# Hevagog/as-cops-and-thieves

Hardware: AMD Instinct MI355X
Metric: env-steps/sec (whole node) at 4096 parallel envs, 2v1 agents, 64-ray sensors (higher is better)
Workload: dtype f64; 1 GPU; 2 cops vs 1 thieves, labyrinth map (30 hull walls / 119 planes), 4096 envs per GPU, 64 rays/agent, dt=1/60, max_step_count=400, Philox random actions, auto-reset; envs_per_gpu=4096, rays=64, agents=3, map=labyrinth, parallelism=env-sharded x1, no data-path collective, episodes_reset_per_gpu=32768, burn_in_steps=600

## Files before the change

### as_cops_and_thieves_amd/csrc/cat_sim_scheduler.h

```cpp
template <class D>
__device__ __forceinline__ Lds carve(const Params &p, char *smem, const MapDesc &md, int slot, int wave)
{
    Lds L;
    const int S = md.S, P = md.P, W = p.wpb;
    L.bb = reinterpret_cast<const double *>(smem);
    L.planes = L.bb + kBB * S;
    L.p32 = reinterpret_cast<const float *>(L.planes + 8 * P);
    L.fc = reinterpret_cast<const int *>(L.planes + geo_rest_doubles(md));
    L.fp = L.fc + S;
    L.rayd = reinterpret_cast<const double *>(smem + p.lds_map_bytes - 16 * D::R(p));
    L.ctrl = reinterpret_cast<int *>(smem + p.lds_map_bytes);
    char *w = smem + p.lds_map_bytes + ctrl_bytes(W) + slot * p.lds_env_bytes;
    const int A = D::A(p), R = D::R(p), NPs = D::NP(p) > 0 ? D::NP(p) : 1;
    L.rec = w;
    double *d = reinterpret_cast<double *>(w);
    L.pos = d; d += 2 * A; L.vel = d; d += 2 * A; L.vb = d; d += 2 * A; L.tc = d; d += 2 * A;
    L.leaf = d; d += 4 * A;
    L.cnt = reinterpret_cast<int *>(d);
    d = reinterpret_cast<double *>(w + D::hot_bytes(p));
    L.wjn = d; d += A * kK; L.pjn = d; d += NPs;
    {
        int *ri = reinterpret_cast<int *>(d);
        L.wsh = ri; ri += A * kK; L.wag = ri; ri += A * kK; L.pag = ri;
    }
// ... 297 lines not shown
            else {
                PHASE(pc, 9);
                physics_env<D>(Ls, p, uni(K->md.S), lane, pc);
                PHASE(pc, 10);
            }
            __builtin_amdgcn_fence(__ATOMIC_RELEASE, "workgroup");
            int d = 0;
            if (lane == 0) {
                d = __hip_atomic_fetch_add(&ctrl[4 * slot + 1], 1, __ATOMIC_RELAXED, __HIP_MEMORY_SCOPE_WORKGROUP);
                c = __hip_atomic_fetch_add(&ctrl[4 * slot + 0], 1, __ATOMIC_RELAXED, __HIP_MEMORY_SCOPE_WORKGROUP);
            }
            d = uni(d); c = uni(c);
            if (d == last_unit) fin_mask |= 1u << slot;
        }
    }
    PHASE(pc, 16);
    if (fin_mask) __builtin_amdgcn_fence(__ATOMIC_ACQUIRE, "workgroup");
    PHASE(pc, 21);
#ifdef CAT_PHASE_TIMING
    bool wb_first = true;
#endif
    while (fin_mask) {
        const int lane = opaque_v(lane0);
        const Params &p = *(const Params *)launder((ParamsK)pp0);
        const LaunchArgs &la = *(const LaunchArgs *)launder(lap0);
        int *const ctrl = reinterpret_cast<int *>(smem + p.lds_map_bytes);
        const BlockDesc *const K = block_desc_lds(smem, p, W);
        const int slot = uni(__builtin_ctz(fin_mask));
        fin_mask &= fin_mask - 1;
        const Lds Ls = carve<D>(p, smem, K->md, slot, wave);
        const int e_s = uni(ctrl[4 * slot + 3]);
        const int step2 = uni(Ls.flags[0]), captured2 = uni(Ls.flags[1]), timeout2 = uni(Ls.flags[2]), rcount = uni(Ls.flags[3]);
        PHASE(pc, 22);
#ifdef CAT_PHASE_TIMING
        asm volatile("s_waitcnt vmcnt(0)" ::: "memory");
        if (wb_first) PHASE(pc, 23); else PHASE(pc, 3);
        wb_first = false;
#endif
        slot_writeback<D>(Ls, p, la, e_s, (long long)e_s, lane, tick, true, step2, captured2, timeout2, rcount, cop_lut, thief_lut, pc);
    }
}

template <class D>
__device__ __forceinline__ void spawn_and_reset(const Lds &L, const Params &p, const LaunchArgs &la, const MapDesc &md,
                                                int env, unsigned rc, int lane);

template <class D>
__device__ __forceinline__ int slot_front(const Lds &L, ParamsK pk, const LaunchArgs &la, const MapDesc &md, const GridDesc &gd,
                                          int env, int lane, int act_pref, unsigned long long synth_tick, int n_fan, PhaseClock &pc)
{
    int captured, timeout, step;
    SetupRow row;
    {
        const Params &p = *(const Params *)launder(pk);
        const int S = md.S, A = D::A(p);
        row = setup_row(L.pos, p, gd, lane, A);
        step = uni(L.cnt[0]) + 1;
        captured = termination_captured<D>(L, p, S, lane);
        timeout = (!captured && step >= p.max_step) ? 1 : 0;
        copy_snapshot(L, A, lane);

        if (lane < A) {
            const int i = lane;
            const double m_inv = 1.0 / p.mass;
            int act;
            if (la.actions) act = act_pref;
            else { unsigned rnd[4]; philox_env(p, env, (unsigned)synth_tick, (unsigned)i, 0xAC710u, rnd); act = (int)(rnd[0] & 3u); }
            if ((unsigned)act > 3u) atomicOr(p.err_word, CAT_DEVERR_BAD_ACTION);
            double jx = 0.0, jy = 0.0;
            if (act == 0) jx = -p.impulse; else if (act == 1) jy = p.impulse;
            else if (act == 2) jx = p.impulse; else if (act == 3) jy = -p.impulse;
            double vx = L.vel[2 * i] + jx * m_inv, vy = L.vel[2 * i + 1] + jy * m_inv;
            double len = sqrt(vx * vx + vy * vy);
            if (len > p.max_speed) { vx = vx / len * p.max_speed; vy = vy / len * p.max_speed; }
            L.vel[2 * i] = vx; L.vel[2 * i + 1] = vy;
        }
        wave_sync();
        PHASE(pc, 2);
    }
    int n_units, rcount = -1, step_store = step;
    {
        const Params &p = *(const Params *)launder(pk);
        n_units = n_fan + 1;
        if (la.auto_reset && (captured || timeout)) {
            physics_env<D>(L, p, uni(md.S), lane, pc);
            rcount = uni(L.cnt[1]) + 1;
            spawn_and_reset<D>(L, p, la, md, env, (unsigned)rcount, lane);
            wave_sync();
            copy_snapshot(L, D::A(p), lane);
            n_units -= 1; step_store = 0;
            row = setup_row(L.fpos, p, gd, lane, D::A(p));
        }
    }
    {
        const Params &p = *(const Params *)launder(pk);
        agent_setup<D>(L, p, gd, lane, row);
        PHASE(pc, 4);
    }
    if (lane == 0) { L.flags[0] = step_store; L.flags[1] = captured; L.flags[2] = timeout; L.flags[3] = rcount; }
    return n_units;
}

constexpr unsigned kRwFinished = 0xFFFFFFFFu;
__device__ __forceinline__ unsigned rw_make(int epoch, int n_units) { return ((unsigned)epoch << 14) | ((unsigned)n_units << 7); }
__device__ __forceinline__ int rw_next(unsigned w) { return (int)(w & 127u); }
__device__ __forceinline__ int rw_units(unsigned w) { return (int)((w >> 7) & 127u); }
__device__ __forceinline__ int rw_epoch(unsigned w) { return (int)(w >> 14); }

__device__ __forceinline__ void lds_release() { __builtin_amdgcn_fence(__ATOMIC_RELEASE, "workgroup", "local"); }
__device__ __forceinline__ void lds_acquire() { __builtin_amdgcn_fence(__ATOMIC_ACQUIRE, "workgroup", "local"); }

template <class D, bool kOneTick>
__device__ __forceinline__ void rollout_body(const Params *__restrict__ pp0, const LaunchArgs &la0)
{
    extern __shared__ __align__(16) char smem[];
    const int lane0 = threadIdx.x % kLanes;
    const int wave = uni(threadIdx.x / kLanes);
    const LaunchArgsK lap0 = kernarg_launch_args();
    PhaseClock pc;
    WSPREAD(0); WSPREAD(4);
    int env, T, W;
    GAS const float *lut_c, *lut_t;
    {
        int uniform;
        const Params q = prologue_params(kernarg_prologue(), uniform);
        const Params &p = *(const Params *)(ParamsK)pp0;
        lut_c = G(q.cop_lut); lut_t = G(q.thief_lut);
        const int lane = lane0;
        W = uni((int)(blockDim.x / kLanes));
        T = kOneTick ? 1 : la0.T;
        WSPREAD(6);
        int *const ctrl = reinterpret_cast<int *>(smem + q.lds_map_bytes);
        BlockDesc bd0;
        prologue_env_desc(q, uniform, W, wave, env, bd0);
        const MapDesc &md0 = bd0.md;
#ifdef CAT_WAVE_SPREAD
        { int e_ = env, s_ = md0.S; asm volatile("" : "+s"(e_), "+v"(s_)); WSPREAD(7); }
#endif
        if (lane < 4) ctrl[4 * wave + lane] = lane == 3 ? env : ((lane == 0 && env < 0) ? (int)kRwFinished : 0);
        StateRegs sregs;
        fetch_state<D>(sregs, q, env, lane);
        stage_map<D>(q, smem, md0, &bd0, const_cast<BlockDesc *>(block_desc_lds(smem, q, W)));
        PHASE(pc, 0);
        WSPREAD(1);
        if (env >= 0) {
            const Lds L = carve<D>(q, smem, md0, wave, wave);
            commit_state<D>(L, sregs, q, lane);
            load_cold<D>(L, p, env, lane);
            PHASE(pc, 1);
        }
    }
    int pend = env >= 0 ? wave : -1, pend_t = 0;
    int hint = wave;
    for (;;) {
        if (pend >= 0) {
            const int lane = opaque_v(lane0);
            const Params &p = *(const Params *)launder((ParamsK)pp0);
            const LaunchArgs &la = *(const LaunchArgs *)launder(lap0);
            int *const ctrl = reinterpret_cast<int *>(smem + p.lds_map_bytes);
            const BlockDesc *const K = block_desc_lds(smem, p, W);
            const int slot = pend, t = pend_t;
            pend = -1;
            SSPREAD(slot, 0);
            const int e_s = uni(ctrl[4 * slot + 3]);
            const Lds Ls = carve<D>(p, smem, K->md, slot, wave);
            int ap = 0;
            if (la.actions && lane < D::A(p)) ap = la.actions[((size_t)t * p.N + e_s) * D::A(p) + lane];
            if (lane == 0) ctrl[4 * slot + 1] = 0;
            const int n_fan = fan_units<D>(p, unit_span<D, kOneTick>(p, K->gd));
#ifndef CAT_ABL_NOFRONT
            const int n2 = slot_front<D>(Ls, (ParamsK)pp0, la, K->md, K->gd, e_s, lane, ap, la.synth_tick + (unsigned long long)t, n_fan, pc);
#else
            const int n2 = n_fan + 1;
            if (lane == 0) { Ls.flags[0] = 1; Ls.flags[1] = 0; Ls.flags[2] = 0; Ls.flags[3] = -1; }
            (void)ap;
#endif
            lds_release();
            if (lane == 0) __hip_atomic_store((unsigned *)&ctrl[4 * slot], rw_make(t + 1, n2), __ATOMIC_RELAXED, __HIP_MEMORY_SCOPE_WORKGROUP);
            hint = slot;
            PHASE(pc, 3);
            WSPREAD(2); SSPREAD(slot, 1);
        }
        int slot, unit, n_units, t;
        {
            const int lane = opaque_v(lane0);
            int *const ctrl = reinterpret_cast<int *>(smem + launder((ParamsK)pp0)->lds_map_bytes);
            unsigned w_l = kRwFinished;
            if (lane < W) w_l = __hip_atomic_load((unsigned *)&ctrl[4 * lane], __ATOMIC_RELAXED, __HIP_MEMORY_SCOPE_WORKGROUP);
            const unsigned open = (unsigned)__ballot(rw_next(w_l) < rw_units(w_l));
            if (open == 0u) {
                if (__ballot(kOneTick ? (w_l == 0u) : (w_l != kRwFinished)) == 0ull) break;
                __builtin_amdgcn_s_sleep(4);
                PHASE(pc, 21);
                continue;
            }
            unsigned key = 0xFFFFFFFFu;
            if (rw_next(w_l) < rw_units(w_l)) key = ((unsigned)rw_epoch(w_l) << 5) | (unsigned)((lane - hint) & 31);
#define CAT_ROW_MIN(SH) { const unsigned o_ = (unsigned)__builtin_amdgcn_update_dpp((int)key, (int)key, 0x120 + SH, 0xF, 0xF, false); key = o_ < key ? o_ : key; }
            CAT_ROW_MIN(8) CAT_ROW_MIN(4) CAT_ROW_MIN(2) CAT_ROW_MIN(1)
#undef CAT_ROW_MIN
            slot = uni((hint + (int)(key & 31u)) & 31);
            const unsigned wv = (unsigned)__builtin_amdgcn_readlane((int)w_l, slot);
            unsigned seen = wv;
            if (lane == 0)
                __hip_atomic_compare_exchange_strong((unsigned *)&ctrl[4 * slot], &seen, wv + 1u, __ATOMIC_RELAXED, __ATOMIC_RELAXED,
                                                     __HIP_MEMORY_SCOPE_WORKGROUP);
            if ((unsigned)uni((int)seen) != wv) continue;
            lds_acquire();
            hint = slot;
            unit = rw_next(wv); n_units = rw_units(wv); t = rw_epoch(wv) - 1;
            PHASE(pc, 22);
        }
        bool fin;
        {
            const int lane = opaque_v(lane0);
            const Params &p = *(const Params *)launder((ParamsK)pp0);
            const LaunchArgs &la = *(const LaunchArgs *)launder(lap0);
            int *const ctrl = reinterpret_cast<int *>(smem + p.lds_map_bytes);
            const BlockDesc *const K = block_desc_lds(smem, p, W);
            const int e_s = uni(ctrl[4 * slot + 3]);
            const Lds Ls = carve<D>(p, smem, K->md, slot, wave);
            const long long eo = (long long)t * p.N + e_s;
            const int gsz = unit_span<D, kOneTick>(p, K->gd);
            SSPREAD(slot, 2 + 2 * unit);
            if (unit < fan_units<D>(p, gsz)) {
#ifndef CAT_ABL_NOFAN
                if constexpr (D::kFan == 1) fan_group<D>(Ls, p, la, K->gd, eo, lane, uni(K->md.S), K->md.cmax, 1, unit, gsz, pc);
                else {
                    const int nch = D::A(p) * ((D::R(p) + kLanes - 1) / kLanes), c0 = unit * gsz, nq = nch - c0 < gsz ? nch - c0 : gsz;
                    unsigned chunks = D::kFixed ? (1u << nq) - 1u : 1u;
                    if (D::kFixed && gsz > 1) chunks = fan_slot<D>(Ls, p, la, K->gd, eo, lane, uni(K->md.S), K->md.cmax, 1, c0, nq, pc);
                    while (chunks) {
                        const int q = uni(__builtin_ctz(chunks));
                        chunks &= chunks - 1;
                        fan_chunk<D>(Ls, p, la, K->gd, eo, lane, uni(K->md.S), K->md.cmax, 1, c0 + q, pc);
                    }
                }
#endif
            } else {
                PHASE(pc, 9);
#ifndef CAT_ABL_NOPHYS
                physics_env<D>(Ls, p, uni(K->md.S), lane, pc);
#endif
                PHASE(pc, 10);
            }
            lds_release();
            SSPREAD(slot, 3 + 2 * unit);
            int d = 0;
            if (lane == 0) d = __hip_atomic_fetch_add(&ctrl[4 * slot + 1], 1, __ATOMIC_RELAXED, __HIP_MEMORY_SCOPE_WORKGROUP);
            fin = uni(d) == n_units - 1;
            PHASE(pc, 23);
        }
        if (!fin) continue;
        {
            const int lane = opaque_v(lane0);
            const Params &p = *(const Params *)launder((ParamsK)pp0);
            const LaunchArgs &la = *(const LaunchArgs *)launder(lap0);
            int *const ctrl = reinterpret_cast<int *>(smem + p.lds_map_bytes);
            const BlockDesc *const K = block_desc_lds(smem, p, W);
            lds_acquire();
            PHASE(pc, 16);
            SSPREAD(slot, 12);
            const int e_s = uni(ctrl[4 * slot + 3]);
            const Lds Ls = carve<D>(p, smem, K->md, slot, wave);
            const long long eo = (long long)t * p.N + e_s;
            const int step2 = uni(Ls.flags[0]), captured2 = uni(Ls.flags[1]), timeout2 = uni(Ls.flags[2]), rcount = uni(Ls.flags[3]);
            const bool last = t + 1 >= T;
#ifndef CAT_ABL_NOWB
            slot_writeback<D>(Ls, p, la, e_s, eo, lane, 1, last, step2, captured2, timeout2, rcount, lut_c, lut_t, pc);
#else
            (void)eo; (void)step2; (void)captured2; (void)timeout2; (void)rcount; (void)la;
#endif
            wave_sync();
            SSPREAD(slot, 13);
            if (!last) { pend = slot; pend_t = t + 1; }
            else if (lane == 0) __hip_atomic_store((unsigned *)&ctrl[4 * slot], kRwFinished, __ATOMIC_RELAXED, __HIP_MEMORY_SCOPE_WORKGROUP);
        }
    }
    PHASE(pc, 11);
    WSPREAD(3); WSPREAD(5);
    pc.flush(lane0);
}

template <class D>
__global__ __launch_bounds__(kMaxWaves *kLanes) void rollout_kernel(const Params *__restrict__ pp0, const LaunchArgs la0, const Prologue)
{
    rollout_body<D, false>(pp0, la0);
}

template <class D>
__global__ __launch_bounds__(kMaxWaves *kLanes) void step_kernel(const Params *__restrict__ pp0, const LaunchArgs la0, const Prologue)
{
    rollout_body<D, true>(pp0, la0);
}

#ifdef CAT_WB_COUNTS
__device__ unsigned long long g_wb_counts[8];
extern "C" int cat_debug_wb_counts(unsigned long long *out8, int reset)
{
    unsigned long long h[8];
    if (hipMemcpyFromSymbol(h, HIP_SYMBOL(g_wb_counts), sizeof h) != hipSuccess) return -1;
    for (int i = 0; i < 8; i++) out8[i] = h[i];
    if (reset) { memset(h, 0, sizeof h); if (hipMemcpyToSymbol(HIP_SYMBOL(g_wb_counts), h, sizeof h) != hipSuccess) return -1; }
    return 0;
}
#endif
template <class T> __device__ __forceinline__ T *slot_ptr(T *p0, int sl, int envb) { return (T *)((char *)const_cast<typename std::remove_const<T>::type *>(p0) + sl * envb); }
constexpr unsigned kPoolValid = 0x80000000u;
constexpr double kPoolEmptyRows = 0.05;
#ifndef CAT_POOL_ROUND
#define CAT_POOL_ROUND 60
#endif
#ifndef CAT_POOL_MIN_PARTIAL
#define CAT_POOL_MIN_PARTIAL 40
#endif
#ifndef CAT_POOL_PATIENCE
#define CAT_POOL_PATIENCE 3
#endif
constexpr int kPoolRound = CAT_POOL_ROUND;
constexpr int kPoolMinPartial = CAT_POOL_MIN_PARTIAL;
constexpr int kPoolPatience = CAT_POOL_PATIENCE;
#ifdef CAT_FAULT_INJECT
constexpr int kSpinLimit = 1 << 14;
#else
constexpr int kSpinLimit = 1 << 22;
#endif
__device__ __forceinline__ int *pool_ctl(char *smem, const Params &p, int W) { return reinterpret_cast<int *>(smem + p.lds_map_bytes + 16 * W + kWgConstBytes - 8); }
static_assert(sizeof(BlockDesc) <= kWgConstBytes - 8, "the pool counters live behind the BlockDesc");

template <bool kExact>
__device__ __forceinline__ int ring_pos(const Params &p, unsigned i)
{
    if constexpr (!kExact) return (int)(i & (unsigned)p.pool_mask);
    const unsigned t = __umulhi(p.pool_magic, i);
    const unsigned q = (t + ((i - t) >> 1)) >> p.pool_shift;
    return (int)(i - q * (unsigned)(p.pool_mask + 1));
}

template <class D, bool kExact>
__device__ __forceinline__ int pool_sort(const Lds &L, const Params &p, const LaunchArgs &la, const GridDesc &gd, long long env, int slot, int lane,
                                         int *pctl, unsigned long long *pool)
{
    const int A = D::A(p), R = D::R(p);
    const unsigned d_empty = f64_to_f16(p.ray_length);
    const unsigned long long lt_mask = (1ull << lane) - 1ull;
    const int cpa = (R + kLanes - 1) / kLanes, nch = A * cpa;
    const int my_cell = lane < A ? L.acell[lane] : -1;
    const int my_dk0 = lane < A * A ? L.dk0[lane] : 0, my_dcnt = lane < A * A ? L.dcnt[lane] : 0;
    int n_res = 0;
    for (int c0 = 0; c0 < nch; c0 += 4) {
        unsigned wrow[4] = {0u, 0u, 0u, 0u};
#pragma unroll
        for (int q = 0; q < 4; q++) {
            if (c0 + q < nch) {
                const int i = (c0 + q) / cpa, k = ((c0 + q) - i * cpa) * kLanes + lane;
                const int cell = __builtin_amdgcn_readlane(my_cell, i);
                const size_t r = (cell < 0 || k >= R) ? 0 : (size_t)cell * R + k;
                wrow[q] = ((GAS const unsigned *)G(p.grid_rows))[gd.row_base + r];
            }
        }
#pragma unroll
        for (int q = 0; q < 4; q++) {
            if (c0 + q < nch) {
                const int i = (c0 + q) / cpa, k = ((c0 + q) - i * cpa) * kLanes + lane;
                const int cell = __builtin_amdgcn_readlane(my_cell, i);
                const bool in = k < R;
                const unsigned rowv = (in && cell >= 0) ? wrow[q] : 0u;
                unsigned dynmask = 0;
                if (in)
                    for (int j = 0; j < A; j++) {
                        if (j == i) continue;
                        const int dc = __builtin_amdgcn_readlane(my_dcnt, i * A + j) & 0xFFFF, dk = __builtin_amdgcn_readlane(my_dk0, i * A + j);
                        int rel = k - dk; if (rel < 0) rel += R;
                        if (rel < dc) dynmask |= 1u << j;
                    }
                bool act = rowv != 0u || dynmask != 0u;
                const unsigned long long m = __ballot(act);
                const int n = __popcll(m);
                int base = 0;
                if (n) {
                    if (lane == 0) base = __hip_atomic_fetch_add(&pctl[1], n, __ATOMIC_RELAXED, __HIP_MEMORY_SCOPE_WORKGROUP);
                    base = uni(base);
                }
                unsigned long long *const e = &pool[act ? ring_pos<kExact>(p, (unsigned)(base + __popcll(m & lt_mask))) : 0];
#ifdef CAT_FAULT_INJECT
                if (slot == 0 && c0 + q == 0 && n && lane == (int)__builtin_ctzll(m)) act = false;
#endif
                for (int spins = 0; __ballot(act && __hip_atomic_load(e, __ATOMIC_RELAXED, __HIP_MEMORY_SCOPE_WORKGROUP) != 0ull) != 0ull;)
                    if (++spins >= kSpinLimit) { if (lane == 0) atomicOr(p.err_word, CAT_DEVERR_SCHEDULER); break; }
                if (act) {
                    const unsigned meta = kPoolValid | ((unsigned)slot << 24) | ((unsigned)i << 16) | (dynmask << 8) | (unsigned)k;
                    __hip_atomic_store(e, ((unsigned long long)meta << 32) | rowv, __ATOMIC_RELAXED, __HIP_MEMORY_SCOPE_WORKGROUP);
                } else if (in && (rowv == 0u && dynmask == 0u)) {
                    const int o = i * R + k;
                    L.od[o] = (unsigned short)d_empty;
                    L.ot[o] = (unsigned char)CAT_EMPTY;
                    if (la.out.hit_shape) la.out.hit_shape[(size_t)env * A * R + o] = -1;
                }
                n_res += __popcll(__ballot(in && (rowv == 0u && dynmask == 0u)));
            }
        }
    }
    return n_res;
}

template <class D, bool kExact>
__device__ __forceinline__ unsigned pool_round(const Lds &L0, const Params &p, const LaunchArgs &la, int S, float cmax, int base, int n, int lane, int *ctrl,
                               unsigned long long *pool, PhaseClock &pc)
{
    const int A = D::A(p), R = D::R(p), envb = p.lds_env_bytes;
    const double r2 = p.ray_radius;
    const unsigned d_empty = f64_to_f16(p.ray_length);
    const unsigned long long lt_mask = (1ull << lane) - 1ull;
    const int gate = launder(uni(p.gate)), n_cops = launder(uni(D::n_cops(p)));
    const double wall_r = launder(p.wall_r), rc = launder(p.rc);
    const int idb = launder(uni(p.row_id_bits)), cmul = launder(uni(p.row_cnt_mul));
    auto row_count = [&](unsigned w) -> int { return w ? (((31 - __builtin_clz(w)) * cmul) >> 16) + 1 : 0; };
    bool on = lane < n;
    unsigned w0 = 0u, meta = 0u;
    if (on) {
        unsigned long long *e = &pool[ring_pos<kExact>(p, (unsigned)(base + lane))];
        unsigned long long v = 0ull;
        int spins = 0;
        do { v = __hip_atomic_load(e, __ATOMIC_RELAXED, __HIP_MEMORY_SCOPE_WORKGROUP); } while (!(v >> 63) && ++spins < kSpinLimit);
        if (!(v >> 63)) { atomicOr(p.err_word, CAT_DEVERR_SCHEDULER); on = false; }
        __hip_atomic_store(e, 0ull, __ATOMIC_RELAXED, __HIP_MEMORY_SCOPE_WORKGROUP);
        w0 = (unsigned)v; meta = (unsigned)(v >> 32);
    }
    lds_acquire();
    const int s = (int)((meta >> 24) & 15u), i = (int)((meta >> 16) & 7u), k = (int)(meta & 255u);
    const unsigned dynmask = on ? ((meta >> 8) & 255u) : 0u;
    if (!on) w0 = 0u;
    unsigned *const rlist = L0.arow;
    rlist[lane] = meta;
    const double *const fpos = slot_ptr(L0.fpos, s, envb), *const ftc = slot_ptr(L0.ftc, s, envb), *const fleaf = slot_ptr(L0.fleaf, s, envb);
    const double2 org = *reinterpret_cast<const double2 *>(fpos + 2 * i);
    const double ax = org.x, ay = org.y;
    const int cnt_w = row_count(w0);
    const int cnt = cnt_w + __popc(dynmask);
    double rdx, rdy, rix, riy;
    {
        const double bx = ax + L0.rayd[2 * k], by = ay + L0.rayd[2 * k + 1];
        rdx = bx - ax; rdy = by - ay; rix = 1.0 / rdx; riy = 1.0 / rdy;
    }
    double best_a = 1.0;
    int best_fi = -1;
    int jj0 = 0;
    wave_sync();
    PHASE(pc, 20);
    while (__ballot(cnt > jj0) != 0ull) {
        int n_items = 0, jj = jj0;
        for (; jj < jj0 + kPassJ; jj++) {
            const bool has = cnt > jj;
            if (__ballot(has) == 0ull) break;
            int id = 0;
            double tbb = 0.0;
            if (has) {
                if (jj < cnt_w) id = (int)((w0 >> (idb * jj)) & ((1u << idb) - 1u)) - 1;
                else {
                    unsigned dj = dynmask;
                    for (int q = jj - cnt_w; q > 0; q--) dj &= dj - 1;
                    id = S + __builtin_ctz(dj);
                }
                if (gate) tbb = bb_segment_query((id < S) ? (L0.bb + kBB * id) : (fleaf + 4 * (id - S)), ax, ay, rdx, rdy, rix, riy);
            }
            const bool live = has && tbb < best_a;
            const unsigned long long m = __ballot(live);
            const int c = __popcll(m);
            if (n_items + c > kItemCap) break;
            int t = 0xFFFF;
            if (live) {
                t = n_items + __popcll(m & lt_mask);
                L0.itm[t] = (unsigned short)(lane | (id << 6));
                L0.itbb[t] = tbb;
            }
            L0.itemidx[(jj - jj0) * kLanes + lane] = (unsigned short)t;
            n_items += c;
        }
        const int jj1 = jj;
        wave_sync();
        PHASE(pc, 5);
        for (int t0 = 0; t0 < n_items; t0 += kLanes) {
            const int t = t0 + lane;
            if (t < n_items) {
                const int d = L0.itm[t];
                const int il = d & 63, id = (d >> 6) & 63;
                const unsigned m2 = rlist[il];
                const int s2 = (int)((m2 >> 24) & 15u), ia = (int)((m2 >> 16) & 7u), k2 = (int)(m2 & 255u);
                const double *const fpos2 = slot_ptr(L0.fpos, s2, envb), *const ftc2 = slot_ptr(L0.ftc, s2, envb);
                const double2 o2 = *reinterpret_cast<const double2 *>(fpos2 + 2 * ia);
                const double cbx = o2.x + L0.rayd[2 * k2], cby = o2.y + L0.rayd[2 * k2 + 1];
                double alpha = 2.0;
                int feat = 0;
                {
                    const bool wall = id < S;
                    const int j = wall ? 0 : id - S;
                    const int *const an2 = slot_ptr(L0.anear, s2, envb);
                    const bool inside = wall ? (id == an2[2 * ia] || id == an2[2 * ia + 1]) : ((((unsigned)slot_ptr(L0.adn, s2, envb)[ia] >> j) & 1u) != 0u);
                    if (inside) { alpha = 0.0; feat = kFeatNear; }
                    else {
                        int f;
                        poly_query_feat(L0, cmax, wall, wall ? id : 0, wall ? wall_r : rc, ftc2[2 * j], ftc2[2 * j + 1], o2.x, o2.y, cbx, cby, r2, alpha, f);
                        feat = f < 0 ? 0 : f;
                    }
                }
                L0.ialpha[t] = alpha; L0.itm[t] = (unsigned short)((id << 6) | feat);
            }
        }
        wave_sync();
        PHASE(pc, 6);
        for (int q = jj0; q < jj1; q++) {
            const int t = cnt > q ? (int)L0.itemidx[(q - jj0) * kLanes + lane] : 0xFFFF;
            if (t != 0xFFFF) {
                const double al = L0.ialpha[t];
                if (al < best_a && L0.itbb[t] < best_a) { best_a = al; best_fi = L0.itm[t]; }
            }
        }
        wave_sync();
        PHASE(pc, 7);
        jj0 = jj1;
    }
    unsigned d16 = d_empty, ty = CAT_EMPTY;
    int best = -1;
    if (best_fi >= 0) {
        const double bx = ax + L0.rayd[2 * k], by = ay + L0.rayd[2 * k + 1];
        best = best_fi >> 6;
        const int f = best_fi & 63;
        const double t = best_a;
        double px = bx, py = by;
        if (f != kFeatNear) {
            const bool wall = best < S;
            const int fc = wall ? L0.fc[best] : 0, first = fc & 0xFFFF, count = fc >> 16;
            if (wall && f < count) {
                const double2 nn = *reinterpret_cast<const double2 *>(L0.planes + 8 * (first + f));
                px = (ax * (1.0 - t) + bx * t) - nn.x * r2;
                py = (ay * (1.0 - t) + by * t) - nn.y * r2;
            } else {
                double2 v = *reinterpret_cast<const double2 *>(L0.planes + 8 * (first + (wall ? f - count : 0)) + 2);
                if (!wall) { v.x = ftc[2 * (best - S)]; v.y = ftc[2 * (best - S) + 1]; }
                circle_hit_point(v.x, v.y, ax, ay, bx, by, t, r2, px, py);
            }
        }
        d16 = obs_distance_f16(px, py, ax, ay);
        ty = (best < S) ? CAT_WALL : ((best - S) >= n_cops ? CAT_THIEF : CAT_COP);
    }
    if (on) {
        const int o = i * R + k;
        slot_ptr(L0.od, s, envb)[o] = (unsigned short)d16;
        slot_ptr(L0.ot, s, envb)[o] = (unsigned char)ty;
        if (la.out.hit_shape) {
            const long long eo = (long long)(rw_epoch((unsigned)ctrl[4 * s]) - 1) * p.N + ctrl[4 * s + 3];
            la.out.hit_shape[(size_t)eo * A * R + o] = best;
        }
        const unsigned want = i < n_cops ? CAT_THIEF : CAT_COP;
        if (ty == want) __hip_atomic_fetch_min(&slot_ptr(L0.dmin, s, envb)[i], d16, __ATOMIC_RELAXED, __HIP_MEMORY_SCOPE_WORKGROUP);
    }
    PHASE(pc, 8);
    lds_release();
    bool fin = false;
    if (on) fin = __hip_atomic_fetch_add(&ctrl[4 * s + 1], 1, __ATOMIC_RELAXED, __HIP_MEMORY_SCOPE_WORKGROUP) + 1 == A * R + 1;
    unsigned long long fm = __ballot(fin);
    unsigned done = 0u;
    while (fm) {
        const int l = __builtin_ctzll(fm);
        fm &= fm - 1;
        done |= 1u << __builtin_amdgcn_readlane(s, l);
    }
    return done;
}

template <class D, bool kOneTick, bool kExact>
__device__ __forceinline__ void rollout_body_pool(const Params *__restrict__ pp0, const LaunchArgs &la0)
{
    extern __shared__ __align__(16) char smem[];
    const int lane0 = threadIdx.x % kLanes;
    const int wave = uni(threadIdx.x / kLanes);
    const LaunchArgsK lap0 = kernarg_launch_args();
    PhaseClock pc;
    WSPREAD(0); WSPREAD(4);
    int env, T, W;
    GAS const float *lut_c, *lut_t;
    {
        int uniform;
        const Params q = prologue_params(kernarg_prologue(), uniform);
        const Params &p = *(const Params *)(ParamsK)pp0;
        lut_c = G(q.cop_lut); lut_t = G(q.thief_lut);
        const int lane = lane0;
        W = uni((int)(blockDim.x / kLanes));
        T = kOneTick ? 1 : la0.T;
        WSPREAD(6);
        int *const ctrl = reinterpret_cast<int *>(smem + q.lds_map_bytes);
        BlockDesc bd0;
        prologue_env_desc(q, uniform, W, wave, env, bd0);
        const MapDesc &md0 = bd0.md;
#ifdef CAT_WAVE_SPREAD
        { int e_ = env, s_ = md0.S; asm volatile("" : "+s"(e_), "+v"(s_)); WSPREAD(7); }
#endif
        if (lane < 4) ctrl[4 * wave + lane] = lane == 3 ? env : ((lane == 0 && env < 0) ? (int)kRwFinished : 0);
        {
            u32x4 *pz = reinterpret_cast<u32x4 *>(smem + q.lds_pool_off);
            const u32x4 z = {0u, 0u, 0u, 0u};
            for (int o = threadIdx.x; o < (q.pool_mask + 1) / 2; o += blockDim.x) pz[o] = z;
            if (threadIdx.x == 0) { int *pc2 = pool_ctl(smem, q, W); pc2[0] = 0; pc2[1] = 0; }
        }
        StateRegs sregs;
        fetch_state<D>(sregs, q, env, lane);
        stage_map<D>(q, smem, md0, &bd0, const_cast<BlockDesc *>(block_desc_lds(smem, q, W)));
        PHASE(pc, 0);
        WSPREAD(1);
        if (env >= 0) {
            const Lds L = carve<D>(q, smem, md0, wave, wave);
            commit_state<D>(L, sregs, q, lane);
            load_cold<D>(L, p, env, lane);
            PHASE(pc, 1);
        }
    }
    unsigned todo = env >= 0 ? 1u << wave : 0u;
    unsigned wbm = 0u;
    int hint = wave, idle = 0;
    int stall = 0, moved_sig = 0;
    unsigned w_seen = 0u;
    for (;;) {
        while (todo) {
            const int lane = opaque_v(lane0);
            const Params &p = *(const Params *)launder((ParamsK)pp0);
            const LaunchArgs &la = *(const LaunchArgs *)launder(lap0);
            int *const ctrl = reinterpret_cast<int *>(smem + p.lds_map_bytes);
            const BlockDesc *const K = block_desc_lds(smem, p, W);
            const int slot = uni(__builtin_ctz(todo));
            todo &= todo - 1;
            SSPREAD(slot, 0);
            const int e_s = uni(ctrl[4 * slot + 3]), t = uni(ctrl[4 * slot + 2]);
            const Lds Ls = carve<D>(p, smem, K->md, slot, wave);
            int ap = 0;
            if (la.actions && lane < D::A(p)) ap = la.actions[((size_t)t * p.N + e_s) * D::A(p) + lane];
            if (lane == 0) ctrl[4 * slot + 1] = 0;
            const int n2 = slot_front<D>(Ls, (ParamsK)pp0, la, K->md, K->gd, e_s, lane, ap, la.synth_tick + (unsigned long long)t, 0, pc);
            lds_release();
            if (lane == 0) __hip_atomic_store((unsigned *)&ctrl[4 * slot], rw_make(t + 1, n2), __ATOMIC_RELAXED, __HIP_MEMORY_SCOPE_WORKGROUP);
            PHASE(pc, 3);
            const int n_res = pool_sort<D, kExact>(Ls, p, la, K->gd, (long long)t * p.N + e_s, slot, lane, pool_ctl(smem, p, W), reinterpret_cast<unsigned long long *>(smem + p.lds_pool_off));
            lds_release();
            const int add = n_res + (n2 == 0 ? 1 : 0);
            int old = 0;
            if (lane == 0) old = __hip_atomic_fetch_add(&ctrl[4 * slot + 1], add, __ATOMIC_RELAXED, __HIP_MEMORY_SCOPE_WORKGROUP);
            if (add > 0 && uni(old) + add == D::A(p) * D::R(p) + 1) wbm |= 1u << slot;
            hint = slot;
            WSPREAD(2); SSPREAD(slot, 1);
        }
#ifdef CAT_WB_COUNTS
        if (wbm && lane0 == 0) { const int k_ = __popc(wbm); atomicAdd(&g_wb_counts[k_ > 7 ? 7 : k_], 1ull); }
#endif
        while (wbm) {
            const int lane = opaque_v(lane0);
            const Params &p = *(const Params *)launder((ParamsK)pp0);
            const LaunchArgs &la = *(const LaunchArgs *)launder(lap0);
            int *const ctrl = reinterpret_cast<int *>(smem + p.lds_map_bytes);
            const BlockDesc *const K = block_desc_lds(smem, p, W);
            const int slot = uni(__builtin_ctz(wbm));
            wbm &= wbm - 1;
            lds_acquire();
            PHASE(pc, 16);
            SSPREAD(slot, 12);
            const int e_s = uni(ctrl[4 * slot + 3]), t = uni(ctrl[4 * slot + 2]);
            const Lds Ls = carve<D>(p, smem, K->md, slot, wave);
            const long long eo = (long long)t * p.N + e_s;
            const int step2 = uni(Ls.flags[0]), captured2 = uni(Ls.flags[1]), timeout2 = uni(Ls.flags[2]), rcount = uni(Ls.flags[3]);
            const bool last = t + 1 >= T;
            slot_writeback<D>(Ls, p, la, e_s, eo, lane, 1, last, step2, captured2, timeout2, rcount, lut_c, lut_t, pc);
            wave_sync();
            SSPREAD(slot, 13);
            if (!last) { if (lane == 0) ctrl[4 * slot + 2] = t + 1; todo |= 1u << slot; }
            else if (lane == 0) __hip_atomic_store((unsigned *)&ctrl[4 * slot], kRwFinished, __ATOMIC_RELAXED, __HIP_MEMORY_SCOPE_WORKGROUP);
        }
        if (todo) continue;
        int base, n, slot = -1;
        {
            const int lane = opaque_v(lane0);
            const Params &p = *(const Params *)launder((ParamsK)pp0);
            int *const ctrl = reinterpret_cast<int *>(smem + p.lds_map_bytes);
            int *const pctl = pool_ctl(smem, p, W);
            unsigned w_l = kRwFinished;
            if (lane < W) w_l = __hip_atomic_load((unsigned *)&ctrl[4 * lane], __ATOMIC_RELAXED, __HIP_MEMORY_SCOPE_WORKGROUP);
            int hd = 0, tl = 0;
            if (lane == 0) { hd = __hip_atomic_load(&pctl[0], __ATOMIC_RELAXED, __HIP_MEMORY_SCOPE_WORKGROUP); tl = __hip_atomic_load(&pctl[1], __ATOMIC_RELAXED, __HIP_MEMORY_SCOPE_WORKGROUP); }
            hd = uni(hd); tl = uni(tl);
            const int avail = tl - hd;
            const unsigned open = (unsigned)__ballot(rw_next(w_l) < rw_units(w_l));
            if (avail >= kPoolRound || (open == 0u && (avail >= kPoolMinPartial || (avail > 0 && idle >= kPoolPatience)))) {
                base = hd; n = avail < kPoolRound ? avail : kPoolRound;
                int seen = hd;
                if (lane == 0) __hip_atomic_compare_exchange_strong(&pctl[0], &seen, hd + n, __ATOMIC_RELAXED, __ATOMIC_RELAXED, __HIP_MEMORY_SCOPE_WORKGROUP);
                if (uni(seen) != hd) continue;
            } else if (open != 0u) {
                n = 0; base = 0;
                unsigned key = 0xFFFFFFFFu;
                if (rw_next(w_l) < rw_units(w_l)) key = ((unsigned)rw_epoch(w_l) << 5) | (unsigned)((lane - hint) & 31);
#define CAT_ROW_MIN(SH) { const unsigned o_ = (unsigned)__builtin_amdgcn_update_dpp((int)key, (int)key, 0x120 + SH, 0xF, 0xF, false); key = o_ < key ? o_ : key; }
                CAT_ROW_MIN(8) CAT_ROW_MIN(4) CAT_ROW_MIN(2) CAT_ROW_MIN(1)
#undef CAT_ROW_MIN
                slot = uni((hint + (int)(key & 31u)) & 31);
                const unsigned wv = (unsigned)__builtin_amdgcn_readlane((int)w_l, slot);
                unsigned seen = wv;
                if (lane == 0)
                    __hip_atomic_compare_exchange_strong((unsigned *)&ctrl[4 * slot], &seen, wv + 1u, __ATOMIC_RELAXED, __ATOMIC_RELAXED, __HIP_MEMORY_SCOPE_WORKGROUP);
                if ((unsigned)uni((int)seen) != wv) continue;
                hint = slot;
            } else {
                if (avail == 0 && __ballot(kOneTick ? (w_l == 0u) : (w_l != kRwFinished)) == 0ull) break;
                ++idle;
                {
                    const bool moved = __ballot(w_l != w_seen) != 0ull || hd + tl != moved_sig;
                    w_seen = w_l; moved_sig = hd + tl;
                    stall = moved ? 0 : stall + 1;
                }
                if (stall > kSpinLimit) { if (lane == 0) atomicOr(p.err_word, CAT_DEVERR_SCHEDULER); break; }
                __builtin_amdgcn_s_sleep(4);
                PHASE(pc, 21);
                continue;
            }
            idle = 0;
            lds_acquire();
            PHASE(pc, 22);
        }
        {
            const int lane = opaque_v(lane0);
            const Params &p = *(const Params *)launder((ParamsK)pp0);
            const LaunchArgs &la = *(const LaunchArgs *)launder(lap0);
            int *const ctrl = reinterpret_cast<int *>(smem + p.lds_map_bytes);
            const BlockDesc *const K = block_desc_lds(smem, p, W);
            if (n > 0) {
                const Lds L0 = carve<D>(p, smem, K->md, 0, wave);
                wbm |= pool_round<D, kExact>(L0, p, la, uni(K->md.S), K->md.cmax, base, n, lane, ctrl, reinterpret_cast<unsigned long long *>(smem + p.lds_pool_off), pc);
            } else {
                const Lds Ls = carve<D>(p, smem, K->md, slot, wave);
                SSPREAD(slot, 2);
                PHASE(pc, 9);
                physics_env<D>(Ls, p, uni(K->md.S), lane, pc);
                PHASE(pc, 10);
                lds_release();
                SSPREAD(slot, 3);
                int old = 0;
                if (lane == 0) old = __hip_atomic_fetch_add(&ctrl[4 * slot + 1], 1, __ATOMIC_RELAXED, __HIP_MEMORY_SCOPE_WORKGROUP);
                if (uni(old) + 1 == D::A(p) * D::R(p) + 1) wbm |= 1u << slot;
            }
            PHASE(pc, 23);
        }
    }
    PHASE(pc, 11);
    WSPREAD(3); WSPREAD(5);
    pc.flush(lane0);
}

template <class D, bool kExact = false>
__global__ __launch_bounds__(kMaxWaves *kLanes) void rollout_kernel_pooled(const Params *__restrict__ pp0, const LaunchArgs la0, const Prologue)
{
    rollout_body_pool<D, false, kExact>(pp0, la0);
}
template <class D, bool kExact = false>
__global__ __launch_bounds__(kMaxWaves *kLanes) void step_kernel_pooled(const Params *__restrict__ pp0, const LaunchArgs la0, const Prologue)
{
    rollout_body_pool<D, true, kExact>(pp0, la0);
}

template <class D>
__device__ __forceinline__ void reset_slot(const Lds &L, const Params &p, const LaunchArgs &la, const MapDesc &md,
                                           const GridDesc &gd, int env, int wave, int lane);

template <class D>
__global__ __launch_bounds__(kMaxWaves *kLanes) void reset_kernel(const Params *__restrict__ pp0, const LaunchArgs la0, const Prologue)
{
    extern __shared__ __align__(16) char smem[];
    const int lane0 = threadIdx.x % kLanes;
    const int wave = uni(threadIdx.x / kLanes);
    const LaunchArgsK lap0 = kernarg_launch_args();
    PhaseClock pc;
    int W;
    {
        const Params &p = *pp0;
        int uniform;
        const Params q = prologue_params(kernarg_prologue(), uniform);
        const int lane = lane0;
        W = uni((int)(blockDim.x / kLanes));
        int env;
        BlockDesc bd0;
        prologue_env_desc(q, uniform, W, wave, env, bd0);
        bool need = env >= 0;
        if (need) {
            if (la0.use_done_mask)
                need = ((GAS const int *)(G(q.state) + (size_t)env * D::rec_bytes(q) + 96 * D::A(q)))[2] != 0;
            else if (la0.mask) need = la0.mask[env] != 0;
        }
        if (!__syncthreads_or(need ? 1 : 0)) return;
        const MapDesc &md0 = bd0.md;
        const GridDesc &gd0 = bd0.gd;
        int *const ctrl = reinterpret_cast<int *>(smem + q.lds_map_bytes);
        if (lane < 4) ctrl[4 * wave + lane] = lane == 3 ? (need ? env : -1) : 0;
        stage_map<D>(q, smem, md0, &bd0, const_cast<BlockDesc *>(block_desc_lds(smem, q, W)));
        if (need) {
            const Lds L = carve<D>(p, smem, md0, wave, wave);
            reset_slot<D>(L, p, la0, md0, gd0, env, wave, lane);
        }
    }
    run_units<D>(pp0, lap0, smem, W, wave, lane0, 0, pc);
}

template <class D>
__device__ __forceinline__ void reset_slot(const Lds &L, const Params &p, const LaunchArgs &la, const MapDesc &md,
                                           const GridDesc &gd, int env, int wave, int lane)
{
    const int A = D::A(p);
    load_state<D>(L, p, env, lane);
    const unsigned rc = (unsigned)(uni(L.cnt[1]) + 1);
    spawn_and_reset<D>(L, p, la, md, env, rc, lane);
    wave_sync();
    copy_snapshot(L, A, lane);
    agent_setup<D>(L, p, gd, lane, setup_row(L.fpos, p, gd, lane, A));
    if (lane == 0) { L.flags[0] = 0; L.flags[1] = 0; L.flags[2] = 0; L.flags[3] = (int)rc; }
    publish_slot(L, wave, lane, fan_units<D>(p));
}

template <class D>
__device__ __forceinline__ void spawn_and_reset(const Lds &L, const Params &p, const LaunchArgs &la, const MapDesc &md,
                                                int env, unsigned rc, int lane)
{
    const int S = md.S, A = D::A(p);
    GAS const double *start = G(p.geo_f64) + md.f64_off + 4 * md.S + geo_rest_doubles(md);
    GAS const double *regions = start + 2 * md.A;
// ... 92 lines not shown
```

Baseline: 134.9 million env-steps/s.

## Process each lane's first candidate in-register and skip empty compaction passes

Each ray lane now tests its first candidate polygon directly in registers (own) instead of pushing it through the LDS item compaction pool. The compaction, alpha evaluation and reduction phases are merged into one loop, and wave_syncs and LDS writes are skipped when a pass produces no pooled items. A per-pass bitmask limits the reduction to rows that had live items. The aim is to cut LDS traffic and barriers for the common case of one or few candidates per ray. The cost is more divergence and register pressure in the merged loop. It also adds optional debug counters.

```diff
diff --git a/as_cops_and_thieves_amd/csrc/cat_sim_scheduler.h b/as_cops_and_thieves_amd/csrc/cat_sim_scheduler.h
--- a/as_cops_and_thieves_amd/csrc/cat_sim_scheduler.h
+++ b/as_cops_and_thieves_amd/csrc/cat_sim_scheduler.h
@@ -623,6 +623,22 @@
     if (hipMemcpyFromSymbol(h, HIP_SYMBOL(g_wb_counts), sizeof h) != hipSuccess) return -1;
     for (int i = 0; i < 8; i++) out8[i] = h[i];
     if (reset) { memset(h, 0, sizeof h); if (hipMemcpyToSymbol(HIP_SYMBOL(g_wb_counts), h, sizeof h) != hipSuccess) return -1; }
+    return 0;
+}
+#endif
+#ifdef CAT_POOL_COUNTS
+__device__ unsigned long long g_pool_counts[8];
+__device__ __forceinline__ void pool_count(int id, bool v)
+{
+    const unsigned long long m = __ballot(v);
+    if (m && (int)(threadIdx.x % 64) == (int)__builtin_ctzll(__ballot(true))) atomicAdd(&g_pool_counts[id], (unsigned long long)__popcll(m));
+}
+extern "C" int cat_debug_pool_counts(unsigned long long *out8, int reset)
+{
+    unsigned long long h[8];
+    if (hipMemcpyFromSymbol(h, HIP_SYMBOL(g_pool_counts), sizeof h) != hipSuccess) return -1;
+    for (int i = 0; i < 8; i++) out8[i] = h[i];
+    if (reset) { memset(h, 0, sizeof h); if (hipMemcpyToSymbol(HIP_SYMBOL(g_pool_counts), h, sizeof h) != hipSuccess) return -1; }
     return 0;
 }
 #endif
@@ -759,18 +775,30 @@
     const double ax = org.x, ay = org.y;
     const int cnt_w = row_count(w0);
     const int cnt = cnt_w + __popc(dynmask);
-    double rdx, rdy, rix, riy;
-    {
-        const double bx = ax + L0.rayd[2 * k], by = ay + L0.rayd[2 * k + 1];
-        rdx = bx - ax; rdy = by - ay; rix = 1.0 / rdx; riy = 1.0 / rdy;
-    }
+    const double bx = ax + L0.rayd[2 * k], by = ay + L0.rayd[2 * k + 1];
+    const double rdx = bx - ax, rdy = by - ay, rix = 1.0 / rdx, riy = 1.0 / rdy;
     double best_a = 1.0;
     int best_fi = -1;
-    int jj0 = 0;
-    wave_sync();
     PHASE(pc, 20);
-    while (__ballot(cnt > jj0) != 0ull) {
+    const int id0 = cnt_w > 0 ? (int)(w0 & ((1u << idb) - 1u)) - 1 : S + __builtin_ctz(dynmask);
+    bool own = false;
+    double tbb0 = 0.0;
+    if (cnt > 0) {
+        if (gate) tbb0 = bb_segment_query((id0 < S) ? (L0.bb + kBB * id0) : (fleaf + 4 * (id0 - S)), ax, ay, rdx, rdy, rix, riy);
+        own = tbb0 < 1.0;
+    }
+    double alpha0 = 2.0;
+    int feat0 = 0;
+    const bool live0 = own;
+#ifdef CAT_POOL_COUNTS
+    pool_count(0, lane == 0); pool_count(1, on); pool_count(2, on && cnt == 1); pool_count(3, live0);
+    bool cn_more = false;
+#endif
+    int jj0 = 1;
+    for (bool first = true;; first = false) {
+        if (!first && __ballot(cnt > jj0) == 0ull) break;
         int n_items = 0, jj = jj0;
+        unsigned jm = 0u;
         for (; jj < jj0 + kPassJ; jj++) {
             const bool has = cnt > jj;
             if (__ballot(has) == 0ull) break;
@@ -789,28 +817,44 @@
             const unsigned long long m = __ballot(live);
             const int c = __popcll(m);
             if (n_items + c > kItemCap) break;
-            int t = 0xFFFF;
-            if (live) {
-                t = n_items + __popcll(m & lt_mask);
-                L0.itm[t] = (unsigned short)(lane | (id << 6));
-                L0.itbb[t] = tbb;
-            }
-            L0.itemidx[(jj - jj0) * kLanes + lane] = (unsigned short)t;
+            if (c) {
+                int t = 0xFFFF;
+                if (live) {
+                    t = n_items + __popcll(m & lt_mask);
+                    L0.itm[t] = (unsigned short)(lane | (id << 6));
+                    L0.itbb[t] = tbb;
+                }
+                L0.itemidx[(jj - jj0) * kLanes + lane] = (unsigned short)t;
+                jm |= 1u << (jj - jj0);
+            }
+#ifdef CAT_POOL_COUNTS
+            cn_more |= live;
+            pool_count(7, live);
+#endif
             n_items += c;
         }
         const int jj1 = jj;
-        wave_sync();
         PHASE(pc, 5);
-        for (int t0 = 0; t0 < n_items; t0 += kLanes) {
-            const int t = t0 + lane;
-            if (t < n_items) {
-                const int d = L0.itm[t];
-                const int il = d & 63, id = (d >> 6) & 63;
-                const unsigned m2 = rlist[il];
-                const int s2 = (int)((m2 >> 24) & 15u), ia = (int)((m2 >> 16) & 7u), k2 = (int)(m2 & 255u);
-                const double *const fpos2 = slot_ptr(L0.fpos, s2, envb), *const ftc2 = slot_ptr(L0.ftc, s2, envb);
-                const double2 o2 = *reinterpret_cast<const double2 *>(fpos2 + 2 * ia);
-                const double cbx = o2.x + L0.rayd[2 * k2], cby = o2.y + L0.rayd[2 * k2 + 1];
+        if (n_items) wave_sync();
+#ifdef CAT_POOL_COUNTS
+        pool_count(6, lane == 0 && n_items > 0);
+#endif
+        const unsigned long long fm = ~__ballot(own);
+        int t = own ? 0 : __popcll(fm & lt_mask), t_next = __popcll(fm) + lane;
+        while (__ballot(own || t < n_items) != 0ull) {
+            if (own || t < n_items) {
+                double qax = ax, qay = ay, qbx = bx, qby = by;
+                int id = id0, s2 = s, ia = i;
+                if (!own) {
+                    const int d = L0.itm[t];
+                    const int il = d & 63;
+                    id = (d >> 6) & 63;
+                    const unsigned m2 = rlist[il];
+                    s2 = (int)((m2 >> 24) & 15u); ia = (int)((m2 >> 16) & 7u);
+                    const int k2 = (int)(m2 & 255u);
+                    const double2 o2 = *reinterpret_cast<const double2 *>(slot_ptr(L0.fpos, s2, envb) + 2 * ia);
+                    qax = o2.x; qay = o2.y; qbx = o2.x + L0.rayd[2 * k2]; qby = o2.y + L0.rayd[2 * k2 + 1];
+                }
                 double alpha = 2.0;
                 int feat = 0;
                 {
@@ -820,31 +864,41 @@
                     const bool inside = wall ? (id == an2[2 * ia] || id == an2[2 * ia + 1]) : ((((unsigned)slot_ptr(L0.adn, s2, envb)[ia] >> j) & 1u) != 0u);
                     if (inside) { alpha = 0.0; feat = kFeatNear; }
                     else {
+                        const double *const ftc2 = slot_ptr(L0.ftc, s2, envb);
                         int f;
-                        poly_query_feat(L0, cmax, wall, wall ? id : 0, wall ? wall_r : rc, ftc2[2 * j], ftc2[2 * j + 1], o2.x, o2.y, cbx, cby, r2, alpha, f);
+                        poly_query_feat(L0, cmax, wall, wall ? id : 0, wall ? wall_r : rc, ftc2[2 * j], ftc2[2 * j + 1], qax, qay, qbx, qby, r2, alpha, f);
                         feat = f < 0 ? 0 : f;
                     }
                 }
-                L0.ialpha[t] = alpha; L0.itm[t] = (unsigned short)((id << 6) | feat);
-            }
-        }
-        wave_sync();
+                if (own) { alpha0 = alpha; feat0 = feat; }
+                else { L0.ialpha[t] = alpha; L0.itm[t] = (unsigned short)((id << 6) | feat); }
+            }
+            t = t_next; t_next += kLanes;
+            own = false;
+        }
         PHASE(pc, 6);
-        for (int q = jj0; q < jj1; q++) {
-            const int t = cnt > q ? (int)L0.itemidx[(q - jj0) * kLanes + lane] : 0xFFFF;
-            if (t != 0xFFFF) {
-                const double al = L0.ialpha[t];
-                if (al < best_a && L0.itbb[t] < best_a) { best_a = al; best_fi = L0.itm[t]; }
-            }
-        }
-        wave_sync();
+        if (first && live0 && alpha0 < 1.0) { best_a = alpha0; best_fi = (id0 << 6) | feat0; }
+        if (n_items) {
+            wave_sync();
+            for (unsigned mm = jm; mm; mm &= mm - 1u) {
+                const int q = jj0 + __builtin_ctz(mm);
+                const int ti = cnt > q ? (int)L0.itemidx[(q - jj0) * kLanes + lane] : 0xFFFF;
+                if (ti != 0xFFFF) {
+                    const double al = L0.ialpha[ti];
+                    if (al < best_a && L0.itbb[ti] < best_a) { best_a = al; best_fi = L0.itm[ti]; }
+                }
+            }
+            wave_sync();
+        }
         PHASE(pc, 7);
         jj0 = jj1;
     }
+#ifdef CAT_POOL_COUNTS
+    pool_count(4, cn_more); pool_count(5, lane == 0 && __ballot(cnt > 1) != 0ull);
+#endif
     unsigned d16 = d_empty, ty = CAT_EMPTY;
     int best = -1;
     if (best_fi >= 0) {
-        const double bx = ax + L0.rayd[2 * k], by = ay + L0.rayd[2 * k + 1];
         best = best_fi >> 6;
         const int f = best_fi & 63;
         const double t = best_a;
```

Measured after the change: 134.7 million env-steps/s (median of 3 runs). Within noise of the previous version (-0.2%).
